# DCASE-REPO/DESED_task

Hardware: AMD Instinct MI355X
Metric: 10s-clips/sec CRNN mean-teacher train @batch48 (higher is better)
Workload: dtype f32 (fp32 storage and accumulation; the dense contractions of the wide layers run as split-bf16 MFMA, 3 bf16 products per fp32 product, fp32-level accuracy; everything else exact f32)

## Files before the change

### desed_task_amd/csrc/sed_common.h

```cpp
#pragma once

#ifdef SED_EMU
#include "hip_emu.h"
#else
#include <hip/hip_runtime.h>
#define SED_DYN_SMEM(name) extern __shared__ __attribute__((aligned(16))) char name[]
#define SED_LAUNCH(kern, grid, block, smem, stream, ...) \
    hipLaunchKernelGGL(kern, grid, block, smem, stream, __VA_ARGS__)
typedef float f32x16 __attribute__((ext_vector_type(16)));
typedef float f32x4 __attribute__((ext_vector_type(4)));
typedef short s16x8 __attribute__((ext_vector_type(8)));
#endif

#include <stdint.h>

#define SED_API extern "C" __attribute__((visibility("default")))

#define SED_MAX_SMEM(kern, bytes) \
    (void)hipFuncSetAttribute((const void*)(kern), hipFuncAttributeMaxDynamicSharedMemorySize, (int)(bytes))

__global__ __launch_bounds__(256) static void sed_zero4_kernel(float* p0, int n0, float* p1, int n1, float* p2, int n2, float* p3, int n3) {
    const int i = blockIdx.x * 256 + threadIdx.x;
    if (i < n0) p0[i] = 0.f;
    if (i < n1) p1[i] = 0.f;
// ... 96 lines not shown
#ifdef SED_EMU
    return (unsigned)(((((unsigned long long)hi) << 32) | lo) >> shift);
#else
    return __builtin_amdgcn_alignbit(hi, lo, shift);
#endif
}

template <class T_>
__device__ __forceinline__ void sed_pin(T_& x) {
#ifndef SED_EMU
    asm volatile("" : "+v"(x));
#else
    (void)x;
#endif
}
__device__ __forceinline__ void sed_opaque(int& x) {
#ifndef SED_EMU
    asm volatile("" : "+v"(x));
#else
    (void)x;
#endif
}

__device__ __forceinline__ int sed_wave_uniform(int x) {
#ifdef SED_EMU
    return x;
#else
    return __builtin_amdgcn_readfirstlane(x);
#endif
}

__device__ __forceinline__ void sed_wave_sync() {
#ifdef SED_EMU
    emu_wave_sync();
#else
    __builtin_amdgcn_fence(__ATOMIC_ACQ_REL, "wavefront");
    __builtin_amdgcn_wave_barrier();
#endif
}

__device__ __forceinline__ void bf16_split2(float a, float b, unsigned& hi, unsigned& lo) {
#ifdef SED_EMU
    unsigned short h0, l0, h1, l1;
    bf16_split(a, h0, l0);
    bf16_split(b, h1, l1);
    hi = (unsigned)h0 | ((unsigned)h1 << 16);
    lo = (unsigned)l0 | ((unsigned)l1 << 16);
#else
    typedef float f32x2_t __attribute__((ext_vector_type(2)));
    typedef __bf16 bf16x2_t __attribute__((ext_vector_type(2)));
    const f32x2_t v = {a, b};
    hi = __builtin_bit_cast(unsigned, __builtin_convertvector(v, bf16x2_t));
    const f32x2_t hf = {__uint_as_float(hi << 16), __uint_as_float(hi & 0xFFFF0000u)};
    lo = __builtin_bit_cast(unsigned, __builtin_convertvector(v - hf, bf16x2_t));
#endif
}
struct SedOneProduct {};
template <class... ONE>
constexpr int sed_np() { return sizeof...(ONE) ? 1 : 3; }
__device__ __forceinline__ unsigned bf16_round2(float a, float b) {
#ifdef SED_EMU
    return (unsigned)f32_to_bf16(a) | ((unsigned)f32_to_bf16(b) << 16);
#else
    typedef float f32x2_t __attribute__((ext_vector_type(2)));
    typedef __bf16 bf16x2_t __attribute__((ext_vector_type(2)));
    const f32x2_t v = {a, b};
    return __builtin_bit_cast(unsigned, __builtin_convertvector(v, bf16x2_t));
#endif
}

__device__ __forceinline__ f32x16 f32x16_zero() {
    f32x16 z;
#pragma unroll
    for (int i = 0; i < 16; ++i) z[i] = 0.f;
    return z;
}

__device__ __forceinline__ float sed_quad_xor1(float v) {
#ifdef SED_EMU
    return __shfl_xor(v, 1);
#else
    return __builtin_bit_cast(float, __builtin_amdgcn_update_dpp(0, __builtin_bit_cast(int, v), 0xB1, 0xF, 0xF, true));
#endif
}
__device__ __forceinline__ float sed_quad_xor2(float v) {
#ifdef SED_EMU
    return __shfl_xor(v, 2);
#else
    return __builtin_bit_cast(float, __builtin_amdgcn_update_dpp(0, __builtin_bit_cast(int, v), 0x4E, 0xF, 0xF, true));
#endif
}
__device__ __forceinline__ float sed_row_ror4(float v) {
#ifdef SED_EMU
    return __shfl_xor(v, 4);
#else
    return __builtin_bit_cast(float, __builtin_amdgcn_update_dpp(0, __builtin_bit_cast(int, v), 0x124, 0xF, 0xF, true));
#endif
}
__device__ __forceinline__ float sed_row_ror8(float v) {
#ifdef SED_EMU
    return __shfl_xor(v, 8);
#else
    return __builtin_bit_cast(float, __builtin_amdgcn_update_dpp(0, __builtin_bit_cast(int, v), 0x128, 0xF, 0xF, true));
#endif
}
__device__ __forceinline__ float sed_row16_max(float v) {
    v = fmaxf(v, sed_quad_xor1(v)); v = fmaxf(v, sed_quad_xor2(v));
    v = fmaxf(v, sed_row_ror4(v)); v = fmaxf(v, sed_row_ror8(v));
    return v;
}
__device__ __forceinline__ float sed_row16_sum(float v) {
    v += sed_quad_xor1(v); v += sed_quad_xor2(v);
    v += sed_row_ror4(v); v += sed_row_ror8(v);
    return v;
}
__device__ __forceinline__ float sed_half_mirror(float v) {
#ifdef SED_EMU
    return __shfl_xor(v, 7);
#else
    return __builtin_bit_cast(float, __builtin_amdgcn_update_dpp(0, __builtin_bit_cast(int, v), 0x141, 0xF, 0xF, true));
#endif
}
__device__ __forceinline__ float sed_quad_sum(float v) {
    v += sed_quad_xor1(v);
    v += sed_quad_xor2(v);
    return v;
}

__device__ __forceinline__ float wave_sum(float v) {
#pragma unroll
    for (int m = 32; m >= 1; m >>= 1) v += __shfl_xor(v, m);
    return v;
}
__device__ __forceinline__ float wave_min(float v) {
#pragma unroll
    for (int m = 32; m >= 1; m >>= 1) v = fminf(v, __shfl_xor(v, m));
    return v;
}
__device__ __forceinline__ float wave_max(float v) {
#pragma unroll
    for (int m = 32; m >= 1; m >>= 1) v = fmaxf(v, __shfl_xor(v, m));
    return v;
}

__device__ __forceinline__ uint32_t sed_mix32(uint32_t x) {
    x ^= x >> 16; x *= 0x85EBCA6Bu;
    x ^= x >> 13; x *= 0xC2B2AE35u;
    x ^= x >> 16;
    return x;
}
__device__ __forceinline__ uint32_t sed_hash(uint32_t idx, uint32_t seed) {
#ifdef SED_HASH_V1
    return sed_mix32(idx * 0x9E3779B1u + seed);
#else
    uint32_t x = idx * 0x9E3779B1u + sed_mix32(seed);
    x ^= x >> 15;
    return x * 0x2C1B3C6Du;
#endif
}

__device__ __forceinline__ void sed_specaug_draw(int* __restrict__ bounds, int b, int n, int f_param, int n_freq, int t_param,
                                                 int n_time, uint32_t seed) {
    const int i = n == 1 ? 0 : b;
    const float inv = 1.0f / 16777216.0f;
    int f0 = 0, f1 = 0, t0 = 0, t1 = 0;
    if (f_param >= 1) {
        const float value = (float)(sed_hash(4u * i + 0u, seed) >> 8) * inv * (float)f_param;
        const float min_value = (float)(sed_hash(4u * i + 1u, seed) >> 8) * inv * ((float)n_freq - value);
        f0 = (int)min_value;
        f1 = f0 + (int)value;
    }
    if (t_param >= 1) {
        const float value = (float)(sed_hash(4u * i + 2u, seed) >> 8) * inv * (float)t_param;
        const float min_value = (float)(sed_hash(4u * i + 3u, seed) >> 8) * inv * ((float)n_time - value);
        t0 = (int)min_value;
        t1 = t0 + (int)value;
    }
    bounds[4 * b] = f0; bounds[4 * b + 1] = f1; bounds[4 * b + 2] = t0; bounds[4 * b + 3] = t1;
}
__device__ __forceinline__ bool sed_keep(uint32_t idx, uint32_t seed, uint32_t threshold24) {
    return (sed_hash(idx, seed) >> 8) >= threshold24;
}

__device__ __forceinline__ float sed_sigmoid(float x) { return 1.0f / (1.0f + expf(-x)); }
__device__ __forceinline__ float sed_tanh(float x) { return 1.0f - 2.0f / (expf(2.0f * x) + 1.0f); }

__device__ __forceinline__ float sed_fast_exp(float x) {
#ifdef SED_EMU
    return exp2f(x * 1.44269504088896341f);
#else
    return __builtin_amdgcn_exp2f(x * 1.44269504088896341f);
#endif
}
__device__ __forceinline__ float sed_fast_rcp(float x) {
#ifdef SED_EMU
    return 1.0f / x;
#else
    return __builtin_amdgcn_rcpf(x);
#endif
}
__device__ __forceinline__ float sed_fast_sigmoid(float x) { return sed_fast_rcp(1.0f + sed_fast_exp(-x)); }
__device__ __forceinline__ float sed_fast_tanh(float x) { return 1.0f - 2.0f * sed_fast_rcp(sed_fast_exp(2.0f * x) + 1.0f); }

__device__ __forceinline__ void sed_wave_prio_high() {
#if !defined(SED_EMU) && !defined(SED_NO_SETPRIO)
    __builtin_amdgcn_s_setprio(3);
#endif
}

__device__ __forceinline__ void sed_mfma_prio(int on) {
#if !defined(SED_EMU) && !defined(SED_NO_SETPRIO)
    if (on) __builtin_amdgcn_s_setprio(1); else __builtin_amdgcn_s_setprio(0);
#else
    (void)on;
#endif
}

__device__ __forceinline__ void sed_dma16(const void* gptr, void* lds_wave_base) {
#ifdef SED_EMU
    memcpy((char*)lds_wave_base + 16 * emu_lane(), gptr, 16);
#else
    __builtin_amdgcn_global_load_lds(gptr, (__attribute__((address_space(3))) void*)lds_wave_base, 16, 0, 0);
#endif
}
#ifdef SED_EMU
struct sed_rsrc { const char* base; };
static inline sed_rsrc sed_make_rsrc_tid16(const void* p, unsigned) { return sed_rsrc{(const char*)p}; }
static inline void sed_dma16_tid(sed_rsrc r, unsigned soffset_bytes, void* lds_wave_base) {
    memcpy((char*)lds_wave_base + 16 * emu_lane(), r.base + soffset_bytes + 16 * emu_lane(), 16);
}
#else
typedef __amdgpu_buffer_rsrc_t sed_rsrc;
__device__ __forceinline__ sed_rsrc sed_make_rsrc_tid16(const void* p, unsigned bytes) {
    return __builtin_amdgcn_make_buffer_rsrc((void*)p, (short)16, (int)bytes, 0x00007000 | (1 << 23));
}
__device__ __forceinline__ void sed_dma16_tid(sed_rsrc r, unsigned soffset_bytes, void* lds_wave_base) {
    __builtin_amdgcn_raw_ptr_buffer_load_lds(r, (__attribute__((address_space(3))) void*)lds_wave_base, 16, 0, (int)soffset_bytes, 0, 0);
}
#endif
#ifdef SED_EMU
#define SED_WAIT_VM_LDS(N) do { } while (0)
#else
#define SED_WAIT_VM_LDS(N) do { asm volatile("s_waitcnt vmcnt(" #N ") lgkmcnt(0)" ::: "memory"); __builtin_amdgcn_sched_barrier(0); } while (0)
#endif

__device__ __forceinline__ void sed_phase_barrier() {
#ifdef SED_EMU
    emu_block_barrier();
#else
    __builtin_amdgcn_sched_barrier(0);
    asm volatile("s_barrier" ::: "memory");
    __builtin_amdgcn_sched_barrier(0);
#endif
}
__device__ __forceinline__ void sed_wait_lds() {
#ifndef SED_EMU
    asm volatile("s_waitcnt lgkmcnt(0)" ::: "memory");
    __builtin_amdgcn_sched_barrier(0);
#endif
}

template <int ROWS, int NTHREADS, int MAXF, int NB = 8>
__device__ __forceinline__ bool sed_stage_halo_f4(float* tile, const float* __restrict__ x, const int* __restrict__ bounds, int b, int t0,
                                                  int T, int F, int pitch, float center) {
    const int nq = F >> 2;
    if ((F & 3) || (nq & (nq - 1)) || nq < 1) return false;
    const int sh = 31 - __builtin_clz(nq), total = (ROWS + 2) << sh, tid = threadIdx.x;
    int mf0 = 0, mf1 = 0, mt0 = 0, mt1 = 0;
    if (bounds) { mf0 = bounds[4 * b]; mf1 = bounds[4 * b + 1]; mt0 = bounds[4 * b + 2]; mt1 = bounds[4 * b + 3]; }
    constexpr int NIT = ((ROWS + 2) * (MAXF / 4) + NTHREADS - 1) / NTHREADS, NBB = NIT < NB ? NIT : NB;
#pragma unroll
    for (int u0 = 0; u0 < NIT; u0 += NBB) {
        float4 v[NBB];
#pragma unroll
        for (int k = 0; k < NBB; ++k) {
            const int idx = tid + NTHREADS * (u0 + k), ic = idx < total ? idx : total - 1;
            const int i = ic >> sh, q = ic - (i << sh);
            const int t = t0 - 1 + i, tc = t < 0 ? 0 : (t >= T ? T - 1 : t);
            v[k] = *(const float4*)(x + ((size_t)b * T + tc) * F + 4 * q);
        }
        sed_sched_fence();
#pragma unroll
        for (int k = 0; k < NBB; ++k) { sed_pin(v[k].x); sed_pin(v[k].y); sed_pin(v[k].z); sed_pin(v[k].w); }
#pragma unroll
        for (int k = 0; k < NBB; ++k) {
            const int idx = tid + NTHREADS * (u0 + k);
            if (idx < total) {
                const int i = idx >> sh, q = idx - (i << sh), t = t0 - 1 + i, f = 4 * q;
                const bool rowok = t >= 0 && t < T && !(t >= mt0 && t < mt1);
                float* d = tile + i * pitch + 1 + f;
                d[0] = ((rowok && !(f >= mf0 && f < mf1)) ? v[k].x : 0.f) - center;
                d[1] = ((rowok && !(f + 1 >= mf0 && f + 1 < mf1)) ? v[k].y : 0.f) - center;
                d[2] = ((rowok && !(f + 2 >= mf0 && f + 2 < mf1)) ? v[k].z : 0.f) - center;
                d[3] = ((rowok && !(f + 3 >= mf0 && f + 3 < mf1)) ? v[k].w : 0.f) - center;
            }
        }
    }
    if (tid < 2 * (ROWS + 2)) tile[(tid >> 1) * pitch + ((tid & 1) ? F + 1 : 0)] = 0.f - center;
    return true;
}

typedef float f32x2 __attribute__((ext_vector_type(2)));
__device__ __forceinline__ f32x2 pk_fma(f32x2 a, f32x2 b, f32x2 c) { return __builtin_elementwise_fma(a, b, c); }
```

### desed_task_amd/csrc/sed_gru.hip

```cpp
#include "sed_common.h"

#define GRU_H 128

template <int TA, int TB, int NTN>
__global__ __launch_bounds__(256) void gemm_kernel(const float* __restrict__ A, const float* __restrict__ Bm,
                                                   const float* __restrict__ bias, float* __restrict__ Cm, int M, int N, int K,
                                                   int lda, int ldb, int ldc, int k_per_slice, int atomic) {
    constexpr int BM = 128, BN = 32 * NTN, BK = 32, AP = BK + 1, BNP = BN + 1;
    __shared__ float As[BM * AP];
    __shared__ float Bs[BK * BNP];
    const int tid = threadIdx.x, lane = tid & 63, w = tid >> 6, lo = lane & 31, hi = lane >> 5;
    const int m0 = blockIdx.y * BM, n0 = blockIdx.x * BN;
    const int kbeg = blockIdx.z * k_per_slice, kend = min(K, kbeg + k_per_slice);
    f32x16 acc[NTN];
#pragma unroll
    for (int i = 0; i < NTN; ++i) acc[i] = f32x16_zero();

    for (int k0 = kbeg; k0 < kend; k0 += BK) {
        __syncthreads();
        if (TA == 0) {
            for (int idx = tid; idx < BM * BK; idx += 256) {
                const int m = idx / BK, k = idx - m * BK;
                const int gm = m0 + m, gk = k0 + k;
                As[m * AP + k] = (gm < M && gk < kend) ? A[(size_t)gm * lda + gk] : 0.f;
// ... 312 lines not shown
    constexpr int GV = (GI_F / 4 + NT_ - 1) / NT_;
    float4 greg[GV];
    auto load_chunk = [&](int c) {
#pragma unroll
        for (int u = 0; u < GV; ++u) {
            const int e4 = tid + NT_ * u, s = e4 / (3 * H / 4), q = e4 - s * (3 * H / 4);
            const int step = c * CH + s;
            greg[u] = make_float4(0.f, 0.f, 0.f, 0.f);
            if (e4 < GI_F / 4 && step < T) {
                const int t = dir ? T - 1 - step : step;
                greg[u] = *(const float4*)(gi + (((size_t)b * T + t) * 2 + dir) * 3 * H + 4 * q);
            }
        }
    };
    auto park_chunk = [&](int c) {
#pragma unroll
        for (int u = 0; u < GV; ++u)
            if (tid + NT_ * u < GI_F / 4) *(float4*)(gis + (c & 1) * GI_F + 4 * (tid + NT_ * u)) = greg[u];
    };
    auto flush_chunk = [&](int c) {
        constexpr int PER = 5 * H / 4;
        const float* ob = obuf + (c & 1) * OB_F;
        for (int e4 = tid; e4 < CH * PER; e4 += NT_) {
            const int s = e4 / PER, q = e4 - s * PER;
            const int step = c * CH + s;
            if (step >= T) break;
            const int t = dir ? T - 1 - step : step;
            const float4 v = *(const float4*)(ob + s * OBS + (q / (H / 4)) * OBP + 4 * (q % (H / 4)));
            if (q < H / 4) *(float4*)(out + ((size_t)b * T + t) * 2 * H + dir * H + 4 * q) = v;
            else if (saved) *(float4*)(saved + (((size_t)b * T + t) * 2 + dir) * 4 * H + 4 * (q - H / 4)) = v;
        }
    };
    load_chunk(0);
    park_chunk(0);
    __syncthreads();
    int cur = 0;
    for (int c = 0; c < nchunks; ++c) {
        if (c + 1 < nchunks) load_chunk(c + 1);
        if (c > 0) flush_chunk(c - 1);
        const float* gch = gis + (c & 1) * GI_F;
        float* och = obuf + (c & 1) * OB_F;
        const int nsteps = min(CH, T - c * CH);
        for (int s = 0; s < nsteps; ++s) {
            GRU_TS(0)
            const float gr = gch[s * 3 * H + j], gz = gch[s * 3 * H + H + j], gn = gch[s * 3 * H + 2 * H + j];
            f32x2 pr = {0.f, 0.f}, pz = {0.f, 0.f}, pn = {0.f, 0.f};
            f32x2 qr = {0.f, 0.f}, qz = {0.f, 0.f}, qn = {0.f, 0.f};
#pragma unroll
            for (int kb = 0; kb < KH / 4; kb += HB) {
                float4 hq[HB];
#pragma unroll
                for (int k = 0; k < HB; ++k) hq[k] = GRU_NOREAD ? make_float4(gr, gz, gn, gr) : *(const float4*)(hbuf[cur] + half * HP + 4 * (kb + k));
#ifdef GRU_STAMP
                if (kb == 0) GRU_TS(1)
#endif
#pragma unroll
                for (int k0 = 0; k0 < (GRU_NOFMA ? 1 : HB); ++k0) {
                    const int k = kb + k0;
                    const f32x2 lo2 = {hq[k0].x, hq[k0].y}, hi2 = {hq[k0].z, hq[k0].w};
                    f32x2 wn0, wn1;
                    if (k < WR) { wn0 = wn[2 * (k < WR ? k : 0)]; wn1 = wn[2 * (k < WR ? k : 0) + 1]; }
                    else { const float4 w4 = wls[(k - WR) * NT_ + tid]; wn0 = f32x2{w4.x, w4.y}; wn1 = f32x2{w4.z, w4.w}; }
                    pr = pk_fma(wr[2 * k], lo2, pr); pz = pk_fma(wz[2 * k], lo2, pz); pn = pk_fma(wn0, lo2, pn);
                    if (GRU_ACC6) { qr = pk_fma(wr[2 * k + 1], hi2, qr); qz = pk_fma(wz[2 * k + 1], hi2, qz); qn = pk_fma(wn1, hi2, qn); }
                    else { pr = pk_fma(wr[2 * k + 1], hi2, pr); pz = pk_fma(wz[2 * k + 1], hi2, pz); pn = pk_fma(wn1, hi2, pn); }
                }
                if (HB < KH / 4) sed_sched_fence();
            }
            if (GRU_ACC6) { pr += qr; pz += qz; pn += qn; }
#ifdef GRU_STAMP
            sed_pin(pr); sed_pin(pz); sed_pin(pn);
            GRU_TS(2)
#endif
            float ar = pr.x + pr.y, az = pz.x + pz.y, an = pn.x + pn.y;
            ar = sed_quad_sum(ar); az = sed_quad_sum(az); an = sed_quad_sum(an);
#ifdef GRU_STAMP
            sed_pin(ar); sed_pin(az); sed_pin(an);
            GRU_TS(3)
#endif
            const float r = GRU_NOTRANS ? (gr + ar + br) * 0.01f : sed_fast_sigmoid(gr + ar + br);
            const float z = GRU_NOTRANS ? (gz + az + bz) * 0.01f : sed_fast_sigmoid(gz + az + bz);
            const float hn = an + bn;
            const float n = GRU_NOTRANS ? (gn + r * hn) * 0.01f : sed_fast_tanh(gn + r * hn);
            float hnew = (1.0f - z) * n + z * hprev;
#ifdef GRU_STAMP
            sed_pin(hnew);
            GRU_TS(4)
#endif
            hprev = hnew;
            if (GRU_QSTORE) {
                float* o = och + s * OBS;
                const float v4 = half == 0 ? hnew : half == 1 ? r : half == 2 ? z : n;
                if (!GRU_NOOBUF) o[half * OBP + j] = v4;
                if (half == 0) {
                    hbuf[cur ^ 1][(j / KH) * HP + j % KH] = hnew;
                    if (!GRU_NOOBUF) o[4 * OBP + j] = hn;
                }
            } else if (half == 0) {
                hbuf[cur ^ 1][(j / KH) * HP + j % KH] = hnew;
                float* o = och + s * OBS;
                if (!GRU_NOOBUF) { o[j] = hnew; o[OBP + j] = r; o[2 * OBP + j] = z; o[3 * OBP + j] = n; o[4 * OBP + j] = hn; }
            }
            cur ^= 1;
            GRU_TS(5)
            if (!GRU_NOBAR) __syncthreads();
#ifdef GRU_STAMP
            GRU_TS(6)
            ++ts_step;
#endif
        }
        if (c + 1 < nchunks) park_chunk(c + 1);
        __syncthreads();
    }
    flush_chunk(nchunks - 1);
#ifdef GRU_STAMP
    __syncthreads();
    if (blockIdx.x == 0 && gru_stamp_buf)
        for (int i = tid; i < 2 * 32 * 8; i += NT_) gru_stamp_buf[i] = (&s_ts[0][0][0])[i];
#endif
}
#define GRU_S_H 256
#define GRU_S_NB 48
__host__ __device__ constexpr int gru_s_nstream(int f, int ns) { return f * ns / GRU_S_NB; }
__host__ __device__ constexpr bool gru_s_streamed(int f, int ns) { return gru_s_nstream(f + 1, ns) > gru_s_nstream(f, ns); }
__host__ __device__ constexpr int gru_s_block(int e, int ns) { return (GRU_S_NB * (e + 1) + ns - 1) / ns - 1; }
#define GRU_S_FWD_CH 2
#define GRU_S_FWD_NL 7
#define GRU_S_FWD GRU_S_FWD_CH, 13, GRU_S_FWD_NL, 28, 4
#define GRU_S_BWD_CH 2
#define GRU_S_BWD_NL 6
#define GRU_S_BWD GRU_S_BWD_CH, 10, GRU_S_BWD_NL, 32, 4
template <int CH, int NR, int NL, int NS, int RD>
__global__ __launch_bounds__(4 * GRU_S_H) void gru_fwd_stream_kernel(const float* __restrict__ gi, const float* __restrict__ whh0,
                                                                     const float* __restrict__ whh1, const float* __restrict__ bhh0,
                                                                     const float* __restrict__ bhh1, float* __restrict__ out,
                                                                     float* __restrict__ saved, int B, int T) {
    sed_wave_prio_high();
    constexpr int H = GRU_S_H, NT_ = 4 * H, NB = GRU_S_NB;
    static_assert(NR + NL + NS == NB && NS % RD == 0, "ring slot of element e is e mod RD in every step");
    constexpr int OBP = H + 8, OBS = 5 * OBP;
    constexpr int GI_F = CH * 3 * H, OB_F = CH * OBS;
    __shared__ __attribute__((aligned(16))) float hbuf[2][H];
    SED_DYN_SMEM(smem);
    float* gis = (float*)smem;
    float* obuf = gis + 2 * GI_F;
    float4* wls = (float4*)(obuf + 2 * OB_F);
    const int tid = threadIdx.x, j = tid >> 2, q = tid & 3;
    const int b = blockIdx.x >> 1, dir = blockIdx.x & 1;
    const float* W = dir ? whh1 : whh0;
    const float* bhh = dir ? bhh1 : bhh0;
    const float* Wg[3] = {W, W + H * H, W + 2 * H * H};
    int wo = j * H + 4 * q;
    f32x2 wreg[2 * NR];
    f32x2 ring[2 * RD];
#pragma unroll
    for (int f = 0; f < NB; ++f) {
        const int e = gru_s_nstream(f, NS), r = f - e;
        if (gru_s_streamed(f, NS) && e >= RD) continue;
        const float4 w4 = *(const float4*)(Wg[f % 3] + wo + 16 * (f / 3));
        if (gru_s_streamed(f, NS)) { ring[2 * e] = f32x2{w4.x, w4.y}; ring[2 * e + 1] = f32x2{w4.z, w4.w}; }
        else if (r < NR) { wreg[2 * r] = f32x2{w4.x, w4.y}; wreg[2 * r + 1] = f32x2{w4.z, w4.w}; }
        else wls[(r - NR) * NT_ + tid] = w4;
    }
    float br = bhh[j], bz = bhh[H + j], bn = bhh[2 * H + j];
#pragma unroll
    for (int r = 0; r < 2 * NR; ++r) sed_pin(wreg[r]);
#pragma unroll
    for (int e = 0; e < 2 * RD; ++e) sed_pin(ring[e]);
    sed_pin(br); sed_pin(bz); sed_pin(bn);
    if (tid < H) hbuf[0][tid] = 0.f;
    float hprev = 0.f;
    const int nchunks = (T + CH - 1) / CH;
    constexpr int GV = (GI_F / 4 + NT_ - 1) / NT_;
    float4 greg[GV];
    auto load_chunk = [&](int c) {
#pragma unroll
        for (int u = 0; u < GV; ++u) {
            const int e4 = tid + NT_ * u, s = e4 / (3 * H / 4), p = e4 - s * (3 * H / 4);
            const int step = c * CH + s;
            greg[u] = make_float4(0.f, 0.f, 0.f, 0.f);
            if (e4 < GI_F / 4 && step < T) {
                const int t = dir ? T - 1 - step : step;
                greg[u] = *(const float4*)(gi + (((size_t)b * T + t) * 2 + dir) * 3 * H + 4 * p);
            }
        }
    };
    auto park_chunk = [&](int c) {
#pragma unroll
        for (int u = 0; u < GV; ++u)
            if (tid + NT_ * u < GI_F / 4) *(float4*)(gis + (c & 1) * GI_F + 4 * (tid + NT_ * u)) = greg[u];
    };
    auto flush_chunk = [&](int c) {
        constexpr int PER = 5 * H / 4;
        const float* ob = obuf + (c & 1) * OB_F;
        for (int e4 = tid; e4 < CH * PER; e4 += NT_) {
            const int s = e4 / PER, p = e4 - s * PER;
            const int step = c * CH + s;
            if (step >= T) break;
            const int t = dir ? T - 1 - step : step;
            const float4 v = *(const float4*)(ob + s * OBS + (p / (H / 4)) * OBP + 4 * (p % (H / 4)));
            if (p < H / 4) *(float4*)(out + ((size_t)b * T + t) * 2 * H + dir * H + 4 * p) = v;
            else if (saved) *(float4*)(saved + (((size_t)b * T + t) * 2 + dir) * 4 * H + 4 * (p - H / 4)) = v;
        }
    };
    load_chunk(0);
    park_chunk(0);
    __syncthreads();
    int cur = 0;
    for (int c = 0; c < nchunks; ++c) {
        if (c + 1 < nchunks) load_chunk(c + 1);
        if (c > 0) flush_chunk(c - 1);
        const float* gch = gis + (c & 1) * GI_F;
        float* och = obuf + (c & 1) * OB_F;
        const int nsteps = min(CH, T - c * CH);
        for (int s = 0; s < nsteps; ++s) {
            sed_opaque(wo);
            const float gr = gch[s * 3 * H + j], gz = gch[s * 3 * H + H + j], gn = gch[s * 3 * H + 2 * H + j];
            f32x2 acc[3] = {{0.f, 0.f}, {0.f, 0.f}, {0.f, 0.f}};
            const float* hq = hbuf[cur] + 4 * q;
#pragma unroll
            for (int kb = 0; kb < 16; ++kb) {
                const float4 h4 = *(const float4*)(hq + 16 * kb);
                const f32x2 lo2 = {h4.x, h4.y}, hi2 = {h4.z, h4.w};
#pragma unroll
                for (int g = 0; g < 3; ++g) {
                    const int f = 3 * kb + g, e = gru_s_nstream(f, NS), r = f - e;
                    f32x2 w0, w1;
                    if (gru_s_streamed(f, NS)) {
                        w0 = ring[2 * (e % RD)]; w1 = ring[2 * (e % RD) + 1];
                    } else if (r < NR) {
                        w0 = wreg[2 * (r < NR ? r : 0)]; w1 = wreg[2 * (r < NR ? r : 0) + 1];
                    } else {
                        const float4 w4 = wls[(r - NR) * NT_ + tid];
                        w0 = f32x2{w4.x, w4.y}; w1 = f32x2{w4.z, w4.w};
                    }
                    acc[g] = pk_fma(w0, lo2, acc[g]);
                    acc[g] = pk_fma(w1, hi2, acc[g]);
                    if (gru_s_streamed(f, NS)) {
                        const int fn = gru_s_block((e + RD) % NS, NS);
                        const float4 w4 = *(const float4*)(Wg[fn % 3] + wo + 16 * (fn / 3));
                        ring[2 * (e % RD)] = f32x2{w4.x, w4.y}; ring[2 * (e % RD) + 1] = f32x2{w4.z, w4.w};
                    }
                }
                sed_sched_fence();
            }
            float ar = acc[0].x + acc[0].y, az = acc[1].x + acc[1].y, an = acc[2].x + acc[2].y;
            ar = sed_quad_sum(ar); az = sed_quad_sum(az); an = sed_quad_sum(an);
            const float r = sed_fast_sigmoid(gr + ar + br);
            const float z = sed_fast_sigmoid(gz + az + bz);
            const float hn = an + bn;
            const float n = sed_fast_tanh(gn + r * hn);
            const float hnew = (1.0f - z) * n + z * hprev;
            hprev = hnew;
            float* o = och + s * OBS;
            o[q * OBP + j] = q == 0 ? hnew : q == 1 ? r : q == 2 ? z : n;
            if (q == 0) { hbuf[cur ^ 1][j] = hnew; o[4 * OBP + j] = hn; }
            cur ^= 1;
            __syncthreads();
        }
        if (c + 1 < nchunks) park_chunk(c + 1);
        __syncthreads();
    }
    flush_chunk(nchunks - 1);
}
static inline int gru_lds_claim(int smem) {
    int kb = sed_tuning[SED_TUNE_GRU_LDS_KB];
    if (kb <= 0) return smem;
    if (kb > 156) kb = 156;
    return kb * 1024 > smem ? kb * 1024 : smem;
}

SED_API int sed_gru_fwd(const float* gi, const float* whh0, const float* whh1, const float* bhh0, const float* bhh1,
                           float* out, float* saved, int B, int T, int H, void* stream) {
    if (H != 128 && H != 192 && H != 256) return SED_ERR_UNSUPPORTED;
    if (B <= 0 || T <= 0) return SED_OK;
    if (H == 256) {
        int smem = (2 * GRU_S_FWD_CH * 3 * H + 2 * GRU_S_FWD_CH * 5 * (H + 8)) * 4 + GRU_S_FWD_NL * 4 * H * 16;
        smem = gru_lds_claim(smem);
        SED_MAX_SMEM((gru_fwd_stream_kernel<GRU_S_FWD>), smem);
        SED_LAUNCH((gru_fwd_stream_kernel<GRU_S_FWD>), dim3(2 * B), dim3(4 * H), smem, (hipStream_t)stream, gi, whh0, whh1, bhh0, bhh1, out, saved, B, T);
        return sed_check_launch();
    }
#define GRU_FWD_CASE(h, ch)                                                                                                       \
    if (H == h) {                                                                                                                 \
        int smem = (2 * ch * 3 * h + 2 * ch * 5 * (GRU_QSTORE ? h + 8 : h)) * 4 + (h <= 128 ? 0 : 8 * 4 * h * 16);               \
        smem = gru_lds_claim(smem);                                                                                               \
        SED_MAX_SMEM((gru_fwd_kernel<h, ch>), smem);                                                                              \
        SED_LAUNCH((gru_fwd_kernel<h, ch>), dim3(2 * B), dim3(4 * h), smem, (hipStream_t)stream, gi, whh0, whh1, bhh0, bhh1, out, saved, B, T); \
    }
    GRU_FWD_CASE(128, GRU_CH) GRU_FWD_CASE(192, 4)
#undef GRU_FWD_CASE
    return sed_check_launch();
}

template <int H, int CH>
__global__ __launch_bounds__(4 * H) void gru_bwd_kernel(const float* __restrict__ dout, const float* __restrict__ out,
                                                      const float* __restrict__ saved, const float* __restrict__ whh0,
                                                      const float* __restrict__ whh1, float* __restrict__ dgi,
                                                      float* __restrict__ dgh, float* __restrict__ hprev_out,
                                                      float* __restrict__ bpart, int B, int T) {
    sed_wave_prio_high();
    constexpr int KH = H / 4, NT_ = 4 * H, HB = H <= 128 ? KH / 4 : 2;
    constexpr int WL = H <= 128 ? 0 : 8, WR = KH / 4 - WL;
    constexpr int QP = GRU_HPAD ? KH + 4 : KH, GP = 4 * QP + (GRU_QSTORE ? 8 : 0);
    constexpr int OBP = GRU_QSTORE ? H + 8 : H, OBS = 7 * OBP;
    constexpr int IB_F = CH * 6 * H, OB_F = CH * OBS;
    __shared__ __attribute__((aligned(16))) float gbuf[2][3 * GP];
    SED_DYN_SMEM(smem);
    float* ibuf = (float*)smem;
    float* obuf = ibuf + 2 * IB_F;
    float4* wls = (float4*)(obuf + 2 * OB_F);
    const int tid = threadIdx.x, k = tid >> 2, half = tid & 3;
    const int b = blockIdx.x >> 1, dir = blockIdx.x & 1;
    const float* W = dir ? whh1 : whh0;
    f32x2 wr[KH / 2], wz[KH / 2], wn[2 * WR];
#pragma unroll
    for (int jj = 0; jj < KH / 2; ++jj) {
        const int j = half * KH + 2 * jj;
        wr[jj] = f32x2{W[(size_t)(0 * H + j) * H + k], W[(size_t)(0 * H + j + 1) * H + k]};
        wz[jj] = f32x2{W[(size_t)(1 * H + j) * H + k], W[(size_t)(1 * H + j + 1) * H + k]};
        if (jj < 2 * WR) wn[jj] = f32x2{W[(size_t)(2 * H + j) * H + k], W[(size_t)(2 * H + j + 1) * H + k]};
    }
#pragma unroll
    for (int q = 0; q < WL; ++q) {
        const int j = half * KH + 4 * (WR + q);
        wls[q * NT_ + tid] = make_float4(W[(size_t)(2 * H + j) * H + k], W[(size_t)(2 * H + j + 1) * H + k],
                                         W[(size_t)(2 * H + j + 2) * H + k], W[(size_t)(2 * H + j + 3) * H + k]);
    }
#pragma unroll
    for (int jj = 0; jj < KH / 2; ++jj) { sed_pin(wr[jj]); sed_pin(wz[jj]); if (jj < 2 * WR) sed_pin(wn[jj]); }
    const int nchunks = (T + CH - 1) / CH;
    constexpr int IV = (IB_F / 4 + NT_ - 1) / NT_;
    float4 ireg[IV];
    auto load_chunk = [&](int c) {
#pragma unroll
        for (int u = 0; u < IV; ++u) {
            const int e4 = tid + NT_ * u, s = e4 / (6 * H / 4), q = e4 - s * (6 * H / 4);
            const int rs = c * CH + s;
            ireg[u] = make_float4(0.f, 0.f, 0.f, 0.f);
            if (e4 < IB_F / 4 && rs < T) {
                const int step = T - 1 - rs;
                const int t = dir ? T - 1 - step : step, tp = dir ? t + 1 : t - 1;
                const size_t bt = (size_t)b * T + t;
                if (q < H) ireg[u] = *(const float4*)(saved + (bt * 2 + dir) * 4 * H + 4 * q);
                else if (q < H + H / 4) { if (step > 0) ireg[u] = *(const float4*)(out + ((size_t)b * T + tp) * 2 * H + dir * H + 4 * (q - H)); }
                else ireg[u] = *(const float4*)(dout + bt * 2 * H + dir * H + 4 * (q - H - H / 4));
            }
        }
    };
    auto park_chunk = [&](int c) {
#pragma unroll
        for (int u = 0; u < IV; ++u)
            if (tid + NT_ * u < IB_F / 4) *(float4*)(ibuf + (c & 1) * IB_F + 4 * (tid + NT_ * u)) = ireg[u];
    };
    auto flush_chunk = [&](int c) {
        constexpr int PER = 7 * H / 4;
        const float* ob = obuf + (c & 1) * OB_F;
        for (int e4 = tid; e4 < CH * PER; e4 += NT_) {
            const int s = e4 / PER, q = e4 - s * PER;
            const int rs = c * CH + s;
            if (rs >= T) break;
            const int step = T - 1 - rs;
            const int t = dir ? T - 1 - step : step;
            const size_t bt = (size_t)b * T + t;
            const int pl = q / (H / 4), w4 = 4 * (q - pl * (H / 4));
            const float4 v = *(const float4*)(ob + s * OBS + pl * OBP + w4);
            if (pl < 3) *(float4*)(dgi + (bt * 2 + dir) * 3 * H + pl * H + w4) = v;
            else if (pl == 3) *(float4*)(hprev_out + (bt * 2 + dir) * H + w4) = v;
            else *(float4*)(dgh + (bt * 2 + dir) * 3 * H + (pl - 4) * H + w4) = v;
        }
    };
    load_chunk(0);
    park_chunk(0);
    __syncthreads();
    float dh_carry = 0.f;
    float sb_r = 0.f, sb_z = 0.f, sb_n = 0.f, sb_hn = 0.f;
    int cur = 0;
    for (int c = 0; c < nchunks; ++c) {
        if (c + 1 < nchunks) load_chunk(c + 1);
        if (c > 0) flush_chunk(c - 1);
        const float* ich = ibuf + (c & 1) * IB_F;
        float* och = obuf + (c & 1) * OB_F;
        const int nsteps = min(CH, T - c * CH);
        for (int s = 0; s < nsteps; ++s) {
            const float* in = ich + s * 6 * H;
            const float r = in[k], z = in[H + k], n = in[2 * H + k], hn = in[3 * H + k], hp = in[4 * H + k];
            const float dh = in[5 * H + k] + dh_carry;
            const float dn = dh * (1.0f - z);
            const float dzg = dh * (hp - n);
            const float da_n = dn * (1.0f - n * n);
            const float da_z = dzg * z * (1.0f - z);
            const float da_r = da_n * hn * r * (1.0f - r);
            const float dhn = da_n * r;
            sb_r += da_r; sb_z += da_z; sb_n += da_n; sb_hn += dhn;
            const int gk = (k / KH) * QP + k % KH;
            float* o = och + s * OBS;
            if (GRU_QSTORE) {
                const float g3 = half == 0 ? da_r : half == 1 ? da_z : dhn;
                if (half < 3) gbuf[cur][half * GP + gk] = g3;
                o[half * OBP + k] = half == 0 ? da_r : half == 1 ? da_z : half == 2 ? da_n : hp;
                if (half < 3) o[(4 + half) * OBP + k] = g3;
            } else if (half == 0) {
                gbuf[cur][gk] = da_r; gbuf[cur][GP + gk] = da_z; gbuf[cur][2 * GP + gk] = dhn;
                o[k] = da_r; o[OBP + k] = da_z; o[2 * OBP + k] = da_n; o[3 * OBP + k] = hp;
                o[4 * OBP + k] = da_r; o[5 * OBP + k] = da_z; o[6 * OBP + k] = dhn;
            }
            __syncthreads();
            const float* gv = gbuf[cur] + half * QP;
            f32x2 p0 = {0.f, 0.f}, p1 = {0.f, 0.f}, p2 = {0.f, 0.f};
#pragma unroll
            for (int qb = 0; qb < KH / 4; qb += HB) {
                float4 ga[HB], gc[HB], gd[HB];
#pragma unroll
                for (int q0 = 0; q0 < HB; ++q0) {
                    ga[q0] = *(const float4*)(gv + 4 * (qb + q0));
                    gc[q0] = *(const float4*)(gv + GP + 4 * (qb + q0));
                    gd[q0] = *(const float4*)(gv + 2 * GP + 4 * (qb + q0));
                }
#pragma unroll
                for (int q0 = 0; q0 < HB; ++q0) {
                    const int q4 = qb + q0;
                    const f32x2 a0 = {ga[q0].x, ga[q0].y}, a1 = {ga[q0].z, ga[q0].w};
                    const f32x2 c0 = {gc[q0].x, gc[q0].y}, c1 = {gc[q0].z, gc[q0].w};
                    const f32x2 d0 = {gd[q0].x, gd[q0].y}, d1 = {gd[q0].z, gd[q0].w};
                    f32x2 wn0, wn1;
                    if (q4 < WR) { wn0 = wn[2 * (q4 < WR ? q4 : 0)]; wn1 = wn[2 * (q4 < WR ? q4 : 0) + 1]; }
                    else { const float4 w4 = wls[(q4 - WR) * NT_ + tid]; wn0 = f32x2{w4.x, w4.y}; wn1 = f32x2{w4.z, w4.w}; }
                    p0 = pk_fma(wr[2 * q4], a0, p0); p1 = pk_fma(wz[2 * q4], c0, p1); p2 = pk_fma(wn0, d0, p2);
                    p0 = pk_fma(wr[2 * q4 + 1], a1, p0); p1 = pk_fma(wz[2 * q4 + 1], c1, p1); p2 = pk_fma(wn1, d1, p2);
                }
                if (HB < KH / 4) sed_sched_fence();
            }
            float acc = ((p0.x + p0.y) + (p1.x + p1.y)) + (p2.x + p2.y);
            acc = sed_quad_sum(acc);
            dh_carry = dh * z + acc;
            cur ^= 1;
        }
        __syncthreads();
        if (c + 1 < nchunks) park_chunk(c + 1);
        __syncthreads();
    }
    flush_chunk(nchunks - 1);
    if (bpart != nullptr) {
        float* rec = bpart + (size_t)blockIdx.x * 6 * H;
        if (half == 0) { rec[k] = sb_r; rec[H + k] = sb_z; rec[2 * H + k] = sb_n; }
        if (half == 1) { rec[3 * H + k] = sb_r; rec[4 * H + k] = sb_z; rec[5 * H + k] = sb_hn; }
    }
}
template <int CH, int NR, int NL, int NS, int RD>
__global__ __launch_bounds__(4 * GRU_S_H) void gru_bwd_stream_kernel(const float* __restrict__ dout, const float* __restrict__ out,
                                                                     const float* __restrict__ saved, const float* __restrict__ whh0,
                                                                     const float* __restrict__ whh1, float* __restrict__ dgi,
                                                                     float* __restrict__ dgh, float* __restrict__ hprev_out,
                                                                     float* __restrict__ bpart, int B, int T) {
    sed_wave_prio_high();
    constexpr int H = GRU_S_H, NT_ = 4 * H, NB = GRU_S_NB;
    static_assert(NR + NL + NS == NB && NS % RD == 0, "ring slot of element e is e mod RD in every step");
    constexpr int GP = H + 8;
    constexpr int OBP = H + 8, OBS = 7 * OBP;
    constexpr int IB_F = CH * 6 * H, OB_F = CH * OBS;
    __shared__ __attribute__((aligned(16))) float gbuf[2][3 * GP];
    SED_DYN_SMEM(smem);
    float* ibuf = (float*)smem;
    float* obuf = ibuf + 2 * IB_F;
    float4* wls = (float4*)(obuf + 2 * OB_F);
    __shared__ __attribute__((aligned(16))) float psum[2][H];
    const int tid = threadIdx.x, k = tid >> 2, half = tid & 3;
    const int lane = tid & 63, wv = tid >> 6, grp = 8 * (wv & 7) + (lane >> 3), sl = (lane & 7) + 8 * (wv >> 3);
    const int b = blockIdx.x >> 1, dir = blockIdx.x & 1;
    const float* W = dir ? whh1 : whh0;
    const float* Wg[3] = {W, W + H * H, W + 2 * H * H};
    int wo = sl * H + 4 * grp;
    auto wload = [&](int f) { return *(const float4*)(Wg[f % 3] + wo + 16 * (f / 3) * H); };
    f32x2 wreg[2 * NR];
    f32x2 ring[2 * RD];
#pragma unroll
    for (int f = 0; f < NB; ++f) {
        const int e = gru_s_nstream(f, NS), r = f - e;
        if (gru_s_streamed(f, NS) && e >= RD) continue;
        const float4 w4 = wload(f);
        if (gru_s_streamed(f, NS)) { ring[2 * e] = f32x2{w4.x, w4.y}; ring[2 * e + 1] = f32x2{w4.z, w4.w}; }
        else if (r < NR) { wreg[2 * r] = f32x2{w4.x, w4.y}; wreg[2 * r + 1] = f32x2{w4.z, w4.w}; }
        else wls[(r - NR) * NT_ + tid] = w4;
    }
#pragma unroll
    for (int r = 0; r < 2 * NR; ++r) sed_pin(wreg[r]);
#pragma unroll
    for (int e = 0; e < 2 * RD; ++e) sed_pin(ring[e]);
    const int nchunks = (T + CH - 1) / CH;
    constexpr int IV = (IB_F / 4 + NT_ - 1) / NT_;
    float4 ireg[IV];
    auto load_chunk = [&](int c) {
#pragma unroll
        for (int u = 0; u < IV; ++u) {
            const int e4 = tid + NT_ * u, s = e4 / (6 * H / 4), p = e4 - s * (6 * H / 4);
            const int rs = c * CH + s;
            ireg[u] = make_float4(0.f, 0.f, 0.f, 0.f);
            if (e4 < IB_F / 4 && rs < T) {
                const int step = T - 1 - rs;
                const int t = dir ? T - 1 - step : step, tp = dir ? t + 1 : t - 1;
                const size_t bt = (size_t)b * T + t;
                if (p < H) ireg[u] = *(const float4*)(saved + (bt * 2 + dir) * 4 * H + 4 * p);
                else if (p < H + H / 4) { if (step > 0) ireg[u] = *(const float4*)(out + ((size_t)b * T + tp) * 2 * H + dir * H + 4 * (p - H)); }
                else ireg[u] = *(const float4*)(dout + bt * 2 * H + dir * H + 4 * (p - H - H / 4));
            }
        }
    };
    auto park_chunk = [&](int c) {
#pragma unroll
        for (int u = 0; u < IV; ++u)
            if (tid + NT_ * u < IB_F / 4) *(float4*)(ibuf + (c & 1) * IB_F + 4 * (tid + NT_ * u)) = ireg[u];
    };
    auto flush_chunk = [&](int c) {
        constexpr int PER = 7 * H / 4;
        const float* ob = obuf + (c & 1) * OB_F;
        for (int e4 = tid; e4 < CH * PER; e4 += NT_) {
            const int s = e4 / PER, p = e4 - s * PER;
            const int rs = c * CH + s;
            if (rs >= T) break;
            const int step = T - 1 - rs;
            const int t = dir ? T - 1 - step : step;
            const size_t bt = (size_t)b * T + t;
            const int pl = p / (H / 4), w4 = 4 * (p - pl * (H / 4));
            const float4 v = *(const float4*)(ob + s * OBS + pl * OBP + w4);
            if (pl < 3) *(float4*)(dgi + (bt * 2 + dir) * 3 * H + pl * H + w4) = v;
            else if (pl == 3) *(float4*)(hprev_out + (bt * 2 + dir) * H + w4) = v;
            else *(float4*)(dgh + (bt * 2 + dir) * 3 * H + (pl - 4) * H + w4) = v;
        }
    };
    load_chunk(0);
    park_chunk(0);
    __syncthreads();
    float dh_carry = 0.f;
    float sb_r = 0.f, sb_z = 0.f, sb_n = 0.f, sb_hn = 0.f;
    int cur = 0;
    for (int c = 0; c < nchunks; ++c) {
        if (c + 1 < nchunks) load_chunk(c + 1);
        if (c > 0) flush_chunk(c - 1);
        const float* ich = ibuf + (c & 1) * IB_F;
        float* och = obuf + (c & 1) * OB_F;
        const int nsteps = min(CH, T - c * CH);
        for (int s = 0; s < nsteps; ++s) {
            sed_opaque(wo);
            const float* in = ich + s * 6 * H;
            const float r = in[k], z = in[H + k], n = in[2 * H + k], hn = in[3 * H + k], hp = in[4 * H + k];
            const float dh = in[5 * H + k] + dh_carry;
            const float dn = dh * (1.0f - z);
            const float dzg = dh * (hp - n);
            const float da_n = dn * (1.0f - n * n);
            const float da_z = dzg * z * (1.0f - z);
            const float da_r = da_n * hn * r * (1.0f - r);
            const float dhn = da_n * r;
            sb_r += da_r; sb_z += da_z; sb_n += da_n; sb_hn += dhn;
            float* o = och + s * OBS;
            const float g3 = half == 0 ? da_r : half == 1 ? da_z : dhn;
            if (half < 3) gbuf[cur][half * GP + k] = g3;
            o[half * OBP + k] = half == 0 ? da_r : half == 1 ? da_z : half == 2 ? da_n : hp;
            if (half < 3) o[(4 + half) * OBP + k] = g3;
            __syncthreads();
            const float* gv = gbuf[cur] + sl;
            f32x2 acc[3][2] = {{{0.f, 0.f}, {0.f, 0.f}}, {{0.f, 0.f}, {0.f, 0.f}}, {{0.f, 0.f}, {0.f, 0.f}}};
#pragma unroll
            for (int jb = 0; jb < 16; ++jb) {
#pragma unroll
                for (int g = 0; g < 3; ++g) {
                    const int f = 3 * jb + g, e = gru_s_nstream(f, NS), rr = f - e;
                    const float gj = gv[g * GP + 16 * jb];
                    const f32x2 g2 = {gj, gj};
                    f32x2 w0, w1;
                    if (gru_s_streamed(f, NS)) {
                        w0 = ring[2 * (e % RD)]; w1 = ring[2 * (e % RD) + 1];
                    } else if (rr < NR) {
                        w0 = wreg[2 * (rr < NR ? rr : 0)]; w1 = wreg[2 * (rr < NR ? rr : 0) + 1];
                    } else {
                        const float4 w4 = wls[(rr - NR) * NT_ + tid];
                        w0 = f32x2{w4.x, w4.y}; w1 = f32x2{w4.z, w4.w};
                    }
                    acc[g][0] = pk_fma(w0, g2, acc[g][0]);
                    acc[g][1] = pk_fma(w1, g2, acc[g][1]);
                    if (gru_s_streamed(f, NS)) {
                        const float4 w4 = wload(gru_s_block((e + RD) % NS, NS));
                        ring[2 * (e % RD)] = f32x2{w4.x, w4.y}; ring[2 * (e % RD) + 1] = f32x2{w4.z, w4.w};
                    }
                }
                sed_sched_fence();
            }
            const f32x2 a01 = (acc[0][0] + acc[1][0]) + acc[2][0], a23 = (acc[0][1] + acc[1][1]) + acc[2][1];
            float a0 = sed_quad_sum(a01.x), a1 = sed_quad_sum(a01.y), a2 = sed_quad_sum(a23.x), a3 = sed_quad_sum(a23.y);
            a0 += sed_half_mirror(a0); a1 += sed_half_mirror(a1); a2 += sed_half_mirror(a2); a3 += sed_half_mirror(a3);
            if ((lane & 7) == 0) *(float4*)(psum[wv >> 3] + 4 * grp) = make_float4(a0, a1, a2, a3);
            __syncthreads();
            dh_carry = dh * z + (psum[0][k] + psum[1][k]);
            cur ^= 1;
        }
        __syncthreads();
        if (c + 1 < nchunks) park_chunk(c + 1);
        __syncthreads();
    }
    flush_chunk(nchunks - 1);
    if (bpart != nullptr) {
        float* rec = bpart + (size_t)blockIdx.x * 6 * H;
        if (half == 0) { rec[k] = sb_r; rec[H + k] = sb_z; rec[2 * H + k] = sb_n; }
        if (half == 1) { rec[3 * H + k] = sb_r; rec[4 * H + k] = sb_z; rec[5 * H + k] = sb_hn; }
    }
}
__global__ __launch_bounds__(256) void gru_bias_reduce_kernel(const float* __restrict__ bpart, float* __restrict__ dbi0,
                                                              float* __restrict__ dbi1, float* __restrict__ dbh0,
                                                              float* __restrict__ dbh1, int B, int H) {
    const int j = blockIdx.x * 256 + threadIdx.x, dir = blockIdx.y;
    if (j >= 6 * H) return;
    float s0 = 0.f, s1 = 0.f, s2 = 0.f, s3 = 0.f;
    int b = 0;
    for (; b + 3 < B; b += 4) {
        s0 += bpart[((size_t)2 * b + dir) * 6 * H + j]; s1 += bpart[((size_t)2 * (b + 1) + dir) * 6 * H + j];
        s2 += bpart[((size_t)2 * (b + 2) + dir) * 6 * H + j]; s3 += bpart[((size_t)2 * (b + 3) + dir) * 6 * H + j];
    }
    for (; b < B; ++b) s0 += bpart[((size_t)2 * b + dir) * 6 * H + j];
    const float v = (s0 + s1) + (s2 + s3);
    float* dbi = dir ? dbi1 : dbi0;
    float* dbh = dir ? dbh1 : dbh0;
    if (j < 3 * H) { if (dbi) dbi[j] = v; }
    else if (dbh) dbh[j - 3 * H] = v;
}
SED_API int sed_gru_bwd(const float* dout, const float* out, const float* saved, const float* whh0, const float* whh1,
                           float* dgi, float* dgh, float* hprev, float* dbi0, float* dbi1, float* dbh0, float* dbh1, int B, int T,
                           int H, float* scratch, void* stream) {
    if (H != 128 && H != 192 && H != 256) return SED_ERR_UNSUPPORTED;
    if ((dbi0 == nullptr) != (dbi1 == nullptr) || (dbh0 == nullptr) != (dbh1 == nullptr)) return SED_ERR_ARG;
    const bool want_bias = dbi0 || dbh0;
    if (B <= 0 || T <= 0) {
        if (want_bias) sed_zero4((hipStream_t)stream, dbi0, dbi0 ? 3 * H : 0, dbi1, dbi1 ? 3 * H : 0, dbh0, dbh0 ? 3 * H : 0, dbh1, dbh1 ? 3 * H : 0);
        return SED_OK;
    }
    if (want_bias && scratch == nullptr) return SED_ERR_ARG;
    float* bpart = scratch;
    if (H == 256) {
        int smem = (2 * GRU_S_BWD_CH * 6 * H + 2 * GRU_S_BWD_CH * 7 * (H + 8)) * 4 + GRU_S_BWD_NL * 4 * H * 16;
        smem = gru_lds_claim(smem);
        SED_MAX_SMEM((gru_bwd_stream_kernel<GRU_S_BWD>), smem);
        SED_LAUNCH((gru_bwd_stream_kernel<GRU_S_BWD>), dim3(2 * B), dim3(4 * H), smem, (hipStream_t)stream, dout, out, saved, whh0, whh1, dgi, dgh,
                   hprev, bpart, B, T);
    }
#define GRU_BWD_CASE(h, ch)                                                                                                       \
    if (H == h) {                                                                                                                 \
        int smem = (2 * ch * 6 * h + 2 * ch * 7 * (GRU_QSTORE ? h + 8 : h)) * 4 + (h <= 128 ? 0 : 8 * 4 * h * 16);               \
        smem = gru_lds_claim(smem);                                                                                               \
        SED_MAX_SMEM((gru_bwd_kernel<h, ch>), smem);                                                                              \
        SED_LAUNCH((gru_bwd_kernel<h, ch>), dim3(2 * B), dim3(4 * h), smem, (hipStream_t)stream, dout, out, saved, whh0, whh1, dgi, dgh, \
                   hprev, bpart, B, T);                                                                                           \
    }
    GRU_BWD_CASE(128, GRU_CH) GRU_BWD_CASE(192, 2)
#undef GRU_BWD_CASE
    if (sed_check_launch() != SED_OK) return SED_ERR_LAUNCH;
    if (want_bias)
        SED_LAUNCH(gru_bias_reduce_kernel, dim3((6 * H + 255) / 256, 2), dim3(256), 0, (hipStream_t)stream, (const float*)bpart, dbi0, dbi1,
                   dbh0, dbh1, B, H);
    return sed_check_launch();
}
SED_API int sed_gru_bias_reduce(const float* scratch, float* dbi0, float* dbi1, float* dbh0, float* dbh1, int B, int H, void* stream) {
    if (H != 128 && H != 192 && H != 256) return SED_ERR_UNSUPPORTED;
    if ((dbi0 == nullptr) != (dbi1 == nullptr) || (dbh0 == nullptr) != (dbh1 == nullptr)) return SED_ERR_ARG;
    if (!dbi0 && !dbh0) return SED_OK;
    if (B <= 0) { sed_zero4((hipStream_t)stream, dbi0, dbi0 ? 3 * H : 0, dbi1, dbi1 ? 3 * H : 0, dbh0, dbh0 ? 3 * H : 0, dbh1, dbh1 ? 3 * H : 0); return SED_OK; }
    if (scratch == nullptr) return SED_ERR_ARG;
    SED_LAUNCH(gru_bias_reduce_kernel, dim3((6 * H + 255) / 256, 2), dim3(256), 0, (hipStream_t)stream, scratch, dbi0, dbi1, dbh0, dbh1, B, H);
    return sed_check_launch();
}
```

Baseline: 16740.

## Remap H=128 GRU backward matvec to column-pair ownership with broadcast packed FMA

Result: no change. 16730 (-0.0%).

```diff
diff --git a/desed_task_amd/csrc/sed_common.h b/desed_task_amd/csrc/sed_common.h
--- a/desed_task_amd/csrc/sed_common.h
+++ b/desed_task_amd/csrc/sed_common.h
@@ -422,3 +422,14 @@
 
 typedef float f32x2 __attribute__((ext_vector_type(2)));
 __device__ __forceinline__ f32x2 pk_fma(f32x2 a, f32x2 b, f32x2 c) { return __builtin_elementwise_fma(a, b, c); }
+template <int HI>
+__device__ __forceinline__ f32x2 pk_fma_bcast(f32x2 gg, f32x2 w, f32x2 c) {
+#ifdef SED_EMU
+    const float g = HI ? gg.y : gg.x;
+    return pk_fma(f32x2{g, g}, w, c);
+#else
+    if (HI) asm("v_pk_fma_f32 %0, %1, %2, %0 op_sel:[1,0,0] op_sel_hi:[1,1,1]" : "+v"(c) : "v"(gg), "v"(w));
+    else asm("v_pk_fma_f32 %0, %1, %2, %0 op_sel:[0,0,0] op_sel_hi:[0,1,1]" : "+v"(c) : "v"(gg), "v"(w));
+    return c;
+#endif
+}
diff --git a/desed_task_amd/csrc/sed_gru.hip b/desed_task_amd/csrc/sed_gru.hip
--- a/desed_task_amd/csrc/sed_gru.hip
+++ b/desed_task_amd/csrc/sed_gru.hip
@@ -638,7 +638,9 @@
     sed_wave_prio_high();
     constexpr int KH = H / 4, NT_ = 4 * H, HB = H <= 128 ? KH / 4 : 2;
     constexpr int WL = H <= 128 ? 0 : 8, WR = KH / 4 - WL;
-    constexpr int QP = GRU_HPAD ? KH + 4 : KH, GP = 4 * QP + (GRU_QSTORE ? 8 : 0);
+    constexpr bool PAIR = H == 128;
+    constexpr int NQ = PAIR ? 8 : 4, QR = H / NQ;
+    constexpr int QP = GRU_HPAD ? QR + 4 : QR, GP = NQ * QP + (GRU_QSTORE ? 8 : 0);
     constexpr int OBP = GRU_QSTORE ? H + 8 : H, OBS = 7 * OBP;
     constexpr int IB_F = CH * 6 * H, OB_F = CH * OBS;
     __shared__ __attribute__((aligned(16))) float gbuf[2][3 * GP];
@@ -650,12 +652,22 @@
     const int b = blockIdx.x >> 1, dir = blockIdx.x & 1;
     const float* W = dir ? whh1 : whh0;
     f32x2 wr[KH / 2], wz[KH / 2], wn[2 * WR];
-#pragma unroll
-    for (int jj = 0; jj < KH / 2; ++jj) {
-        const int j = half * KH + 2 * jj;
-        wr[jj] = f32x2{W[(size_t)(0 * H + j) * H + k], W[(size_t)(0 * H + j + 1) * H + k]};
-        wz[jj] = f32x2{W[(size_t)(1 * H + j) * H + k], W[(size_t)(1 * H + j + 1) * H + k]};
-        if (jj < 2 * WR) wn[jj] = f32x2{W[(size_t)(2 * H + j) * H + k], W[(size_t)(2 * H + j + 1) * H + k]};
+    if constexpr (PAIR) {
+        const int j0 = (tid & 7) * QR, p2 = 2 * (tid >> 3);
+#pragma unroll
+        for (int jj = 0; jj < QR; ++jj) {
+            wr[jj] = *(const f32x2*)(W + (size_t)(0 * H + j0 + jj) * H + p2);
+            wz[jj] = *(const f32x2*)(W + (size_t)(1 * H + j0 + jj) * H + p2);
+            wn[jj] = *(const f32x2*)(W + (size_t)(2 * H + j0 + jj) * H + p2);
+        }
+    } else {
+#pragma unroll
+        for (int jj = 0; jj < KH / 2; ++jj) {
+            const int j = half * KH + 2 * jj;
+            wr[jj] = f32x2{W[(size_t)(0 * H + j) * H + k], W[(size_t)(0 * H + j + 1) * H + k]};
+            wz[jj] = f32x2{W[(size_t)(1 * H + j) * H + k], W[(size_t)(1 * H + j + 1) * H + k]};
+            if (jj < 2 * WR) wn[jj] = f32x2{W[(size_t)(2 * H + j) * H + k], W[(size_t)(2 * H + j + 1) * H + k]};
+        }
     }
 #pragma unroll
     for (int q = 0; q < WL; ++q) {
@@ -729,7 +741,7 @@
             const float da_r = da_n * hn * r * (1.0f - r);
             const float dhn = da_n * r;
             sb_r += da_r; sb_z += da_z; sb_n += da_n; sb_hn += dhn;
-            const int gk = (k / KH) * QP + k % KH;
+            const int gk = (k / QR) * QP + k % QR;
             float* o = och + s * OBS;
             if (GRU_QSTORE) {
                 const float g3 = half == 0 ? da_r : half == 1 ? da_z : dhn;
@@ -742,33 +754,62 @@
                 o[4 * OBP + k] = da_r; o[5 * OBP + k] = da_z; o[6 * OBP + k] = dhn;
             }
             __syncthreads();
-            const float* gv = gbuf[cur] + half * QP;
             f32x2 p0 = {0.f, 0.f}, p1 = {0.f, 0.f}, p2 = {0.f, 0.f};
-#pragma unroll
-            for (int qb = 0; qb < KH / 4; qb += HB) {
-                float4 ga[HB], gc[HB], gd[HB];
-#pragma unroll
-                for (int q0 = 0; q0 < HB; ++q0) {
-                    ga[q0] = *(const float4*)(gv + 4 * (qb + q0));
-                    gc[q0] = *(const float4*)(gv + GP + 4 * (qb + q0));
-                    gd[q0] = *(const float4*)(gv + 2 * GP + 4 * (qb + q0));
+            if constexpr (PAIR) {
+                const float* gv = gbuf[cur] + (tid & 7) * QP;
+                float4 ga[QR / 4], gc[QR / 4], gd[QR / 4];
+#pragma unroll
+                for (int q0 = 0; q0 < QR / 4; ++q0) {
+                    ga[q0] = *(const float4*)(gv + 4 * q0);
+                    gc[q0] = *(const float4*)(gv + GP + 4 * q0);
+                    gd[q0] = *(const float4*)(gv + 2 * GP + 4 * q0);
                 }
 #pragma unroll
-                for (int q0 = 0; q0 < HB; ++q0) {
-                    const int q4 = qb + q0;
+                for (int q0 = 0; q0 < QR / 4; ++q0) {
                     const f32x2 a0 = {ga[q0].x, ga[q0].y}, a1 = {ga[q0].z, ga[q0].w};
                     const f32x2 c0 = {gc[q0].x, gc[q0].y}, c1 = {gc[q0].z, gc[q0].w};
                     const f32x2 d0 = {gd[q0].x, gd[q0].y}, d1 = {gd[q0].z, gd[q0].w};
-                    f32x2 wn0, wn1;
-                    if (q4 < WR) { wn0 = wn[2 * (q4 < WR ? q4 : 0)]; wn1 = wn[2 * (q4 < WR ? q4 : 0) + 1]; }
-                    else { const float4 w4 = wls[(q4 - WR) * NT_ + tid]; wn0 = f32x2{w4.x, w4.y}; wn1 = f32x2{w4.z, w4.w}; }
-                    p0 = pk_fma(wr[2 * q4], a0, p0); p1 = pk_fma(wz[2 * q4], c0, p1); p2 = pk_fma(wn0, d0, p2);
-                    p0 = pk_fma(wr[2 * q4 + 1], a1, p0); p1 = pk_fma(wz[2 * q4 + 1], c1, p1); p2 = pk_fma(wn1, d1, p2);
+                    p0 = pk_fma_bcast<0>(a0, wr[4 * q0], p0); p1 = pk_fma_bcast<0>(c0, wz[4 * q0], p1); p2 = pk_fma_bcast<0>(d0, wn[4 * q0], p2);
+                    p0 = pk_fma_bcast<1>(a0, wr[4 * q0 + 1], p0); p1 = pk_fma_bcast<1>(c0, wz[4 * q0 + 1], p1); p2 = pk_fma_bcast<1>(d0, wn[4 * q0 + 1], p2);
+                    p0 = pk_fma_bcast<0>(a1, wr[4 * q0 + 2], p0); p1 = pk_fma_bcast<0>(c1, wz[4 * q0 + 2], p1); p2 = pk_fma_bcast<0>(d1, wn[4 * q0 + 2], p2);
+                    p0 = pk_fma_bcast<1>(a1, wr[4 * q0 + 3], p0); p1 = pk_fma_bcast<1>(c1, wz[4 * q0 + 3], p1); p2 = pk_fma_bcast<1>(d1, wn[4 * q0 + 3], p2);
                 }
-                if (HB < KH / 4) sed_sched_fence();
-            }
-            float acc = ((p0.x + p0.y) + (p1.x + p1.y)) + (p2.x + p2.y);
-            acc = sed_quad_sum(acc);
+            } else {
+                const float* gv = gbuf[cur] + half * QP;
+#pragma unroll
+                for (int qb = 0; qb < KH / 4; qb += HB) {
+                    float4 ga[HB], gc[HB], gd[HB];
+#pragma unroll
+                    for (int q0 = 0; q0 < HB; ++q0) {
+                        ga[q0] = *(const float4*)(gv + 4 * (qb + q0));
+                        gc[q0] = *(const float4*)(gv + GP + 4 * (qb + q0));
+                        gd[q0] = *(const float4*)(gv + 2 * GP + 4 * (qb + q0));
+                    }
+#pragma unroll
+                    for (int q0 = 0; q0 < HB; ++q0) {
+                        const int q4 = qb + q0;
+                        const f32x2 a0 = {ga[q0].x, ga[q0].y}, a1 = {ga[q0].z, ga[q0].w};
+                        const f32x2 c0 = {gc[q0].x, gc[q0].y}, c1 = {gc[q0].z, gc[q0].w};
+                        const f32x2 d0 = {gd[q0].x, gd[q0].y}, d1 = {gd[q0].z, gd[q0].w};
+                        f32x2 wn0, wn1;
+                        if (q4 < WR) { wn0 = wn[2 * (q4 < WR ? q4 : 0)]; wn1 = wn[2 * (q4 < WR ? q4 : 0) + 1]; }
+                        else { const float4 w4 = wls[(q4 - WR) * NT_ + tid]; wn0 = f32x2{w4.x, w4.y}; wn1 = f32x2{w4.z, w4.w}; }
+                        p0 = pk_fma(wr[2 * q4], a0, p0); p1 = pk_fma(wz[2 * q4], c0, p1); p2 = pk_fma(wn0, d0, p2);
+                        p0 = pk_fma(wr[2 * q4 + 1], a1, p0); p1 = pk_fma(wz[2 * q4 + 1], c1, p1); p2 = pk_fma(wn1, d1, p2);
+                    }
+                    if (HB < KH / 4) sed_sched_fence();
+                }
+            }
+            float acc;
+            if constexpr (PAIR) {
+                const f32x2 ps = (p0 + p1) + p2;
+                const float sx = sed_quad_sum(ps.x), sy = sed_quad_sum(ps.y);
+                const bool lowq = (tid & 4) == 0;
+                acc = (lowq ? sx : sy) + sed_half_mirror(lowq ? sy : sx);
+            } else {
+                acc = ((p0.x + p0.y) + (p1.x + p1.y)) + (p2.x + p2.y);
+                acc = sed_quad_sum(acc);
+            }
             dh_carry = dh * z + acc;
             cur ^= 1;
         }
```
